# Vchitect/Latte

Hardware: AMD Instinct MI355X
Metric: denoising steps/sec (higher is better)
Workload: dtype f16; 1 GPU; Latte-XL/2 FaceForensics (uncond) 16x256x256 -> latents 16x4x32x32, DDIM on the '250' respacing, random-init weights; per_gpu_batch=8, global_batch=8, parallelism=dp1 (independent samples)

## Files before the change

### latte_amd/csrc/common.h

```cpp
#pragma once
#include <hip/hip_runtime.h>
#include <stdint.h>
#include <atomic>
#include <string>
#include <vector>

#include "../../include/latte_amd.h"

struct latte_schedule {
  int num_timesteps = 0;
  std::vector<int64_t> timestep_map;
  std::vector<double> betas, alphas_cumprod, alphas_cumprod_prev, alphas_cumprod_next, sqrt_recip_alphas_cumprod,
      sqrt_recipm1_alphas_cumprod, posterior_variance, posterior_log_variance_clipped, posterior_mean_coef1,
      posterior_mean_coef2, log_betas, sqrt_alphas_cumprod, sqrt_one_minus_alphas_cumprod;
  int mean_type = 0;
  int var_type = 0;
  mutable float* dev_tables = nullptr;
  mutable int dev_tables_device = -1;
};
enum DevTable : int { DT_SQRT_AC = 0, DT_SQRT_1MAC, DT_COEF1, DT_COEF2, DT_POST_LOGVAR, DT_LOG_BETAS, DT_SQRT_RECIP, DT_SQRT_RECIPM1,
                      DT_FIXED_LOGVAR, LATTE_NUM_DEV_TABLES };

extern "C" int schedule_device_tables(const latte_schedule_t* s, const float** out, hipStream_t st);

// ... 56 lines not shown
  int gate_stride;
  int rows_per_sample;
  int stagger;
  int group_m;
  int rmw_mode;
  int tag;
  int k_chunk;
  long split_stride;
  const uint8_t* A8;
  const uint8_t* W8;
  const uint8_t* A4;
  const uint8_t* W4;
  const uint8_t* A4s;
  const uint8_t* W4s;
  half_t* aux;
};
constexpr int LO8_A_SHIFT = 12, LO8_W_SHIFT = 6;
inline int lo4_pitch(int K) { return (K + 255) / 256 * 128; }
bool gemm_lo8_ok(int M, int N, int K);
bool gemm_lo4_ok(int M, int N, int K);
int launch_gemm(const GemmArgs& a, int epi, int dtype, int variant, hipStream_t st);
int launch_gemm_pw(const GemmArgs& a, int epi, int dtype, int roll, hipStream_t st);
int gemm_tile_m(int variant);
int gemm_tile_n(int variant);
int gemm_auto_variant(int M, int N, int epi);
int gemm_resolve_variant(int M, int N, int K, int epi);
bool gemm_small_tile_ok(int M, int N, int K);

struct AttnArgs {
  const half_t* qkv;
  half_t* out;
  int num_seq;
// ... 45 lines not shown
                       float* out, int BF, int C, int H, int p, int D, hipStream_t st);
int launch_final_layer(const float* x, const float* shift, const float* scale, int mod_stride,
                       const float* Wt , const float* bias, float* out, int M, int D,
                       int rows_per_sample, int T, int p, int Cout, int H, hipStream_t st);
int launch_cond_rows(const float* temb, const float* ytab, const int64_t* y, float* out, int n_steps, int bu, int D,
                     hipStream_t st);
int launch_text_proj(const float* text, const float* W, const float* bias, float* out, int B, int N, int K, hipStream_t st);
int launch_iota(int64_t* p, int n, hipStream_t st);
int launch_gated_split_reduce(float* x, const float* ws, int splits, size_t stride, const float* bias, const float* gate,
                              int gate_stride, int rows_per_sample, int M, int N, hipStream_t st);
int launch_silu_rows(const float* in, float* out, size_t n, hipStream_t st);
int launch_adaln_single(const float* tables , const float* head_table , const float* t6 ,
                        const float* temb , float* mod, int B, int nblk, int D, hipStream_t st);
int launch_permute_cf(const float* in, float* out, int B, int C, int F, int hw, int to_bfc, hipStream_t st);
int launch_fill_f32(float* p, float v, size_t n, hipStream_t st);
enum DebugChoice { DBG_ATTN_VARIANT = 0, DBG_XATTN_FLASH, DBG_TN_KERNEL, DBG_TN_WN, DBG_ATTN_BWD_TILES, DBG_CONV_KERNEL, DBG_VAE_SPLIT, DBG_NUM_CHOICES };
int debug_choice(DebugChoice c);
int set_debug_choice(const char* name, int value);

int launch_scale_f32(float* p, float s, size_t n, hipStream_t st);
int launch_scale_f32_dev(float* p, const float* s_dev, int inverse, size_t n, hipStream_t st);
int launch_t2v_guided_ddim(float* x, const float* model_out, int b, int C, int Cout, int F, int hw, float scale, float c1, float c2,
                           float c3, float c4, hipStream_t st);
struct T2VLinearStep {
  float scale, m_x, m_eps, c_x, c0, c1, c2, c3, c_noise, in_scale_next;
  int push;
};
int launch_t2v_guided_linear_step(float* x, float* x_in, const float* model_out, const float* h1, const float* h2, const float* h3,
                                  const float* noise, float* hw, int b, int C, int Cout, int F, int HW, const T2VLinearStep& s,
                                  hipStream_t st);
int launch_linear_step(float* x, float* x_in, const float* model_out, const float* h1, const float* h2, const float* h3,
// ... 159 lines not shown
```

### latte_amd/csrc/debug.hip

```cpp
#include "../../include/latte_amd_debug.h"
#include "common.h"

namespace {
typedef __attribute__((ext_vector_type(4))) __bf16 bf16x4;
__global__ void tr16_probe_kernel(uint16_t* out) {
  __shared__ __attribute__((aligned(16))) uint16_t lds[512];
  for (int i = threadIdx.x; i < 512; i += 64) lds[i] = (uint16_t)i;
  __syncthreads();
  const int lane = threadIdx.x;
  auto p = (__attribute__((address_space(3))) bf16x4*)((__attribute__((address_space(3))) char*)lds + 8 * lane);
  bf16x4 v = __builtin_amdgcn_ds_read_tr16_b64_v4bf16(p);
  typedef __attribute__((ext_vector_type(4))) unsigned short u16x4;
  u16x4 u = __builtin_bit_cast(u16x4, v);
  for (int j = 0; j < 4; ++j) out[lane * 4 + j] = u[j];
}

typedef __attribute__((address_space(3))) void lds_void_t;
__global__ void __launch_bounds__(512) dma_probe_kernel(const char* src, long long* out, int mode, int reps) {
  extern __shared__ __attribute__((aligned(16))) char smem[];
  const int lane = threadIdx.x & 63, wave = __builtin_amdgcn_readfirstlane(threadIdx.x >> 6);
  const __amdgpu_buffer_rsrc_t rs = __builtin_amdgcn_make_buffer_rsrc((void*)src, 0, 1u << 30, 0x00020000);
  char* my = smem + wave * 16384;
  const unsigned base = ((blockIdx.x & 63) * 8 + wave) * 16384u;
  long long t_issue = 0, t_all = 0;
// ... 96 lines not shown
extern "C" {

int latte_debug_dma_probe(const void* src_1gib_window, long long* out, int mode, int waves, int reps, void* stream) {
  if (waves < 1 || waves > 8) return fail(LATTE_ERR_INVALID, "dma_probe: waves must be 1..8");
  return launch_lds<dma_probe_kernel>(dim3(256), dim3(64 * waves), 8 * 16384, (hipStream_t)stream, (const char*)src_1gib_window, out, mode,
                                      reps);
}

int latte_debug_gemm(const void* A, const void* W, const float* bias, void* out, const float* gate, int M, int N, int K,
                     int gate_stride, int rows_per_sample, int epi, int dtype, int variant, void* stream) {
  GemmArgs g{};
  g.A = (const half_t*)A; g.W = (const half_t*)W; g.bias = bias; g.out = out; g.gate = gate;
  g.M = M; g.N = N; g.K = K; g.gate_stride = gate_stride; g.rows_per_sample = rows_per_sample;
  if (epi == EPI_BIAS_RES_H16) g.res = (const half_t*)gate;
  if (variant >= 1000) { g.tag = variant / 1000; variant %= 1000; }
  return launch_gemm(g, epi, dtype, variant, (hipStream_t)stream);
}

int latte_debug_gemm_gelu(const void* A, const void* W, const float* bias, void* out, void* aux, int M, int N, int K, int epi, int dtype,
                          void* stream) {
  if (epi != EPI_BIAS_GELU_DUAL_H16 && epi != EPI_DGELU_H16) return fail(LATTE_ERR_INVALID, "gemm_gelu: epi 13 (dual GELU) or 14 (dGELU)");
  GemmArgs g{};
  g.A = (const half_t*)A; g.W = (const half_t*)W; g.bias = bias; g.out = out; g.aux = (half_t*)aux;
  g.M = M; g.N = N; g.K = K; g.rows_per_sample = M;
  return launch_gemm_pw(g, epi, dtype, 1, (hipStream_t)stream);
}

int latte_debug_gemm_lo8(const void* A, const void* W, const void* A8, const void* W8, const float* bias, void* out, const float* gate,
                         int M, int N, int K, int gate_stride, int rows_per_sample, int epi, int dtype, void* stream) {
  if (!A8 || !W8) return fail(LATTE_ERR_INVALID, "gemm_lo8: null fp8 operand");
  GemmArgs g{};
  g.A = (const half_t*)A; g.W = (const half_t*)W; g.bias = bias; g.out = out; g.gate = gate;
  g.M = M; g.N = N; g.K = K; g.gate_stride = gate_stride; g.rows_per_sample = rows_per_sample;
  g.A8 = (const uint8_t*)A8; g.W8 = (const uint8_t*)W8;
  return launch_gemm(g, epi, dtype, 0, (hipStream_t)stream);
}

int latte_debug_gemm_lo4(const void* A, const void* W, const void* A4, const void* A4s, const void* W4, const void* W4s, const float* bias,
                         void* out, const float* gate, int M, int N, int K, int gate_stride, int rows_per_sample, int epi, int dtype,
                         void* stream) {
  if (!A4 || !A4s || !W4 || !W4s) return fail(LATTE_ERR_INVALID, "gemm_lo4: null fp4 operand");
  GemmArgs g{};
  g.A = (const half_t*)A; g.W = (const half_t*)W; g.bias = bias; g.out = out; g.gate = gate;
  g.M = M; g.N = N; g.K = K; g.gate_stride = gate_stride; g.rows_per_sample = rows_per_sample;
  g.A4 = (const uint8_t*)A4; g.A4s = (const uint8_t*)A4s; g.W4 = (const uint8_t*)W4; g.W4s = (const uint8_t*)W4s;
  return launch_gemm(g, epi, dtype, 0, (hipStream_t)stream);
}

int latte_debug_pack_w4(const void* w, void* out4, void* out_scale, int N, int K, int dtype, void* stream) {
  return launch_pack_w4((const half_t*)w, (unsigned char*)out4, (unsigned char*)out_scale, N, K, dtype, (hipStream_t)stream);
}

int latte_debug_ln_modulate_split4(const float* x, void* y, void* y4, void* y4s, const float* shift, const float* scale, int mod_stride, int M,
                                   int D, int rows_per_sample, int dtype, void* stream) {
  return launch_ln_modulate_split4(x, (half_t*)y, (unsigned char*)y4, (unsigned char*)y4s, shift, scale, mod_stride, M, D, rows_per_sample,
                                   dtype, (hipStream_t)stream);
}

int latte_debug_pack_w8(const void* w, void* out8, int64_t n, int dtype, void* stream) {
  return launch_pack_w8((const half_t*)w, (unsigned char*)out8, n, dtype, (hipStream_t)stream);
// ... 698 lines not shown
```

### latte_amd/csrc/engine.cpp

```cpp
#include <algorithm>
#include <cmath>
#include <cstdio>
#include <cstring>
#include <string>
#include <vector>

#include "event_profile.h"
#include "weight_store.h"

namespace latte {

static thread_local std::string g_last_error;
static std::atomic<int> g_debug_choice[DBG_NUM_CHOICES];
int debug_choice(DebugChoice c) { return g_debug_choice[c].load(std::memory_order_relaxed); }
int set_debug_choice(const char* name, int value) {
  static const char* const names[DBG_NUM_CHOICES] = {"attn_variant", "xattn_flash", "tn_kernel", "tn_wn", "attn_bwd_tiles", "conv_kernel", "vae_split"};
  static const int allowed[DBG_NUM_CHOICES][4] = {{1, 5, 12, 13}, {1, 0, 0, 0}, {4, 0, 0, 0}, {4, 0, 0, 0}, {1, 2, 0, 0}, {1, 2, 3, 4}, {0, 0, 0, 0}};
  for (int i = 0; i < DBG_NUM_CHOICES; ++i) {
    if (name && std::string(name) == names[i]) {
      bool ok = value == 0;
      for (int k = 0; k < 4; ++k) ok = ok || (allowed[i][k] != 0 && value == allowed[i][k]);
      ok = ok || (i == DBG_VAE_SPLIT && (value >> 24) == 1);
      if (!ok) return -1;
      g_debug_choice[i].store(value, std::memory_order_relaxed);
      return 0;
    }
  }
  return -1;
}
void set_error(const std::string& msg) { g_last_error = msg; }
int fail(int code, const std::string& msg) {
  g_last_error = msg;
// ... 12 lines not shown

}

using namespace latte;

struct latte_engine {
  latte_model_config_t cfg;
  int max_batch = 0;
  int D = 0, T = 0, F = 0, G = 0, Cin = 0, Cout = 0, H = 0, P = 0, KPE = 0, Hm = 0, hd = 0;
  int nmod = 0;
  int64_t rows_max = 0, rows_pad = 0;
  int gemm_variant = 0;
  int gemm_variant_of[4] = {0, 0, 0, 0};
  int fuse_qkv_attn = 3;
  int gated_split_k = 0;
  int guided_split = 20;
  int guided_split_active = 0;
  bool split_failed = false;
  bool split_w_ready = false;
  hipEvent_t load_event = nullptr;
  half_t* xn2 = nullptr;
  unsigned char* lo8 = nullptr;
  unsigned char *lo4 = nullptr, *lo4s = nullptr;
  float *split_ws = nullptr, *zero_bias = nullptr;
  std::vector<BlockW> blocks;
  float *ada_w = nullptr, *ada_b = nullptr, *pos = nullptr, *temp = nullptr, *pe_wt = nullptr, *pe_b = nullptr,
        *t0_w = nullptr, *t0_b = nullptr, *t2_w = nullptr, *t2_b = nullptr, *ytab = nullptr, *fin_wt = nullptr,
        *fin_b = nullptr;
  float *xres = nullptr, *mod = nullptr, *temb0 = nullptr, *cvec = nullptr, *model_out = nullptr, *noise_buf = nullptr;
  half_t *xn = nullptr, *qkv = nullptr, *hbuf = nullptr;
// ... 30 lines not shown
enum { C_QKV = 0, C_PROJ, C_FC1, C_FC2, C_ATTN_S, C_ATTN_T, C_LN, C_COND, C_PATCH, C_FINAL, C_QKVATTN_S, C_QKVATTN_T, C_NONE = -1 };

constexpr int64_t SPLIT_WS_FLOATS = 256ll * 256 * 192;
int gated_split_choice(const latte_engine* e, int M, int N, int K, int variant) {
  if (variant != 0 || e->gated_split_k == 1 || N % 192 || K % 64) return 1;
  if (e->gated_split_k == 0 && gemm_small_tile_ok(M, N, K)) return 1;
  const int tiles = ((M + 255) / 256) * (N / 192), nk = K / 64;
  if (e->gated_split_k >= 2) {
    const int s = e->gated_split_k;
    return (nk % s == 0 && (int64_t)s * M * N <= SPLIT_WS_FLOATS) ? s : 1;
  }
  for (int s = 4; s >= 2; --s)
    if (tiles * s <= 256 && nk % s == 0 && nk / s >= 32 && (int64_t)s * M * N <= SPLIT_WS_FLOATS) return s;
  return 1;
}
int gated_gemm(latte_engine* e, const GemmArgs& g, int dt, int variant, hipStream_t st) {
  if (g.A8) return launch_gemm(g, EPI_GATE_RES_F32, dt, 0, st);
  const int s = gated_split_choice(e, g.M, g.N, g.K, variant);
  if (s == 1) return launch_gemm(g, EPI_GATE_RES_F32, dt, variant, st);
  GemmArgs p = g;
  p.bias = e->zero_bias;
  p.gate = nullptr;
  p.out = e->split_ws;
  p.k_chunk = g.K / s;
  p.split_stride = (long)g.M * g.N;
  if (int rc = launch_gemm(p, EPI_BIAS_F32, dt, 5, st)) return rc;
  return launch_gated_split_reduce((float*)g.out, e->split_ws, s, (size_t)g.M * g.N, g.bias, g.gate, g.gate_stride,
                                   g.rows_per_sample, g.M, g.N, st);
}

// ... 88 lines not shown
  if ((gsplit & 16) && !gemm_lo4_ok(M, e->Hm, D)) gsplit = (gsplit & ~16) | 8;
  if (gsplit & 16) gsplit &= ~10;
  if (gsplit & 4) gsplit &= ~1;
  if (gsplit & 8) gsplit &= ~2;
  if ((gsplit & 4) && !gemm_lo8_ok(M, D, D)) gsplit = (gsplit & ~4) | 1;
  if ((gsplit & 8) && !gemm_lo8_ok(M, e->Hm, D)) gsplit = (gsplit & ~8) | 2;
  if ((gsplit & 3) && (uint64_t)e->rows_pad * 2 * D * 2 >= (1ull << 32)) gsplit &= ~3;
  if (gsplit) gsplit = ensure_split_weights(e, gsplit, st);
  int gactive = gsplit & 26;

  for (int i = 0; i < c.depth; ++i) {
    const bool spatial = (i % 2) == 0;
    const BlockW& w = e->blocks[i];
    const float* mb = modp + (size_t)i * 6 * D;
    bool split_proj = false;
    const float* te = (i == 1) ? e->temp : nullptr;
    if ((rc = launch_ln_modulate(e->xres, e->xres, e->xn, mb, mb + D, mstride, M, D, rps, te, T, F, dt, st))) return rc;
    tm.mark(C_LN);
    GemmArgs g{};
    g.M = M; g.rows_per_sample = rps; g.gate_stride = mstride;
    const half_t* attn_out = e->xn;
    if (((e->fuse_qkv_attn >> (spatial ? 0 : 1)) & 1) && qkv_attention_fusable(D, c.num_heads, e->hd, F, T, spatial ? 0 : 1, M)) {
      QkvAttnArgs qa{};
      qa.xn = e->xn; qa.w = w.qkv_w; qa.bias = w.qkv_b; qa.out = e->qkv; qa.B = B; qa.F = F; qa.T = T; qa.D = D;
      qa.heads = c.num_heads; qa.hd = e->hd; qa.mode = spatial ? 0 : 1; qa.scale = 1.0f / std::sqrt((float)e->hd);
      qa.flags = ((e->fuse_qkv_attn >> 2) & 7) ^ 7;
      split_proj = gsplit & 5;
      qa.out_split = (gsplit & 4) ? 2 : (gsplit & 1);
      qa.out8 = e->lo8;
      gactive |= gsplit & 5;
      if ((rc = launch_qkv_attention(qa, dt, st))) return rc;
      tm.mark(spatial ? C_QKVATTN_S : C_QKVATTN_T);
      attn_out = e->qkv;
    } else {
      g.A = e->xn; g.W = w.qkv_w; g.bias = w.qkv_b; g.out = e->qkv; g.N = 3 * D; g.K = D;
// ... 20 lines not shown
    tm.mark(C_PROJ);
    const int split_fc1 = (gsplit & 16) ? 3 : (gsplit & 8) ? 2 : (gsplit & 2) ? 1 : 0;
    if (split_fc1 == 3) rc = launch_ln_modulate_split4(e->xres, e->xn, e->lo4, e->lo4s, mb + 3 * D, mb + 4 * D, mstride, M, D, rps, dt, st);
    else rc = launch_ln_modulate(e->xres, e->xres, split_fc1 == 1 ? e->xn2 : e->xn, mb + 3 * D, mb + 4 * D, mstride, M, D, rps, nullptr, T, F, dt, st,
                                 split_fc1, e->lo8);
    if (rc) return rc;
    tm.mark(C_LN);
    g.A = e->xn; g.W = w.fc1_w; g.bias = w.fc1_b; g.out = e->hbuf; g.gate = nullptr; g.N = e->Hm; g.K = D;
    if (split_fc1 == 1) { g.A = e->xn2; g.W = w.fc1_w2; g.K = 2 * D; }
    if (split_fc1 == 2) { g.A8 = e->lo8; g.W8 = w.fc1_w8; }
    if (split_fc1 == 3) { g.A4 = e->lo4; g.A4s = e->lo4s; g.W4 = w.fc1_w4; g.W4s = w.fc1_w4s; }
    if ((rc = launch_gemm(g, EPI_BIAS_GELU_H16, dt, e->gemm_variant_of[2] ? e->gemm_variant_of[2] : e->gemm_variant, st))) return rc;
    g.A8 = nullptr; g.W8 = nullptr; g.A4 = nullptr; g.A4s = nullptr; g.W4 = nullptr; g.W4s = nullptr;
    tm.mark(C_FC1);
    g.A = e->hbuf; g.W = w.fc2_w; g.bias = w.fc2_b; g.out = e->xres; g.gate = mb + 5 * D; g.N = D; g.K = e->Hm; g.tag = 1;

    if ((rc = gated_gemm(e, g, dt, e->gemm_variant_of[3] ? e->gemm_variant_of[3] : e->gemm_variant, st))) return rc;
    tm.mark(C_FC2);
  }
  const float* fm = modp + (size_t)c.depth * 6 * D;
  if ((rc = launch_final_layer(e->xres, fm, fm + D, mstride, e->fin_wt, e->fin_b, out, M, D, rps, T, c.patch_size,
                               e->Cout, e->H, st))) return rc;
  tm.mark(C_FINAL);
  if (cfg_dup) e->guided_split_active = gactive;
  return LATTE_OK;
}

int grow(latte_engine* e, float** p, int64_t* cap, int64_t need) {
  if (*cap >= need) return LATTE_OK;
  if (*p) {
    e->arena.release(*p);
    *p = nullptr;
// ... 260 lines not shown
    return LATTE_OK;
  }
  for (int gi = 0; gi < 4; ++gi) {
    static const char* names[4] = {"gemm_variant_qkv", "gemm_variant_proj", "gemm_variant_fc1", "gemm_variant_fc2"};
    if (k == names[gi]) {
      if (value < 0 || (value > 13 && value != 18 && value != 19)) return fail(LATTE_ERR_INVALID, "gemm_variant_*: must be 0..13, 18 or 19");
      e->gemm_variant_of[gi] = (int)value;
      return LATTE_OK;
    }
  }
  if (k == "gated_split_k") {
    if (value < 0 || value > 4) return fail(LATTE_ERR_INVALID, "gated_split_k: 0 (rule), 1 (off) or 2..4 splits");
    e->gated_split_k = (int)value;
    return LATTE_OK;
  }
  if (k == "fuse_qkv_attn") {
    if (value < 0 || value > 31)
      return fail(LATTE_ERR_INVALID, "fuse_qkv_attn: bit 0 = spatial blocks, bit 1 = temporal blocks, bits 2-4 = schedule features off (0..31)");
    e->fuse_qkv_attn = (int)value;
    return LATTE_OK;
  }
  if (k == "guided_split") {
    if (value < 0 || value > 31)
      return fail(LATTE_ERR_INVALID, "guided_split: bit 0 / 1 = attention output / fc1 operand as f16 split pairs, bit 2 / 3 = the same with an fp8 remainder, bit 4 = fc1's operand with an fp4 remainder, in guided calls (0..31)");
    e->guided_split = (int)value;
    return LATTE_OK;
  }
  if (k == "seed") {
    e->seed = (uint64_t)value;
    e->rng_offset = 0;
// ... 4 lines not shown
    e->train_timesteps = (int)value;
    return LATTE_OK;
  }
  return fail(LATTE_ERR_INVALID, "set_option: unknown option '" + k + "'");
}

int latte_engine_get_option(const latte_engine_t* e, const char* name, int64_t* value) {
  if (!e || !name || !value) return fail(LATTE_ERR_INVALID, "get_option: null argument");
  const std::string k = name;
  if (k == "gemm_variant") *value = e->gemm_variant;
  else if (k == "gemm_variant_qkv") *value = e->gemm_variant_of[0];
  else if (k == "gemm_variant_proj") *value = e->gemm_variant_of[1];
  else if (k == "gemm_variant_fc1") *value = e->gemm_variant_of[2];
  else if (k == "gemm_variant_fc2") *value = e->gemm_variant_of[3];
  else if (k == "gated_split_k") *value = e->gated_split_k;
  else if (k == "fuse_qkv_attn") *value = e->fuse_qkv_attn;
  else if (k == "guided_split") *value = e->guided_split;
  else if (k == "guided_split_active") *value = e->guided_split_active;
  else if (k == "guided_split_failed") *value = e->split_failed ? 1 : 0;
  else if (k == "seed") *value = (int64_t)e->seed;
  else if (k == "train_timesteps") *value = e->train_timesteps;
  else return fail(LATTE_ERR_INVALID, "get_option: unknown option '" + k + "'");
  return LATTE_OK;
}

int latte_engine_load_tensor(latte_engine_t* e, const char* key, const float* data, int64_t numel, int on_device,
                             void* stream) {
  if (!e || !key || !data) return fail(LATTE_ERR_INVALID, "load_tensor: null argument");
  hipStream_t st = (hipStream_t)stream;
  WeightSlot* slot = nullptr;
// ... 544 lines not shown
```

### latte_amd/csrc/gemm.hip

```cpp
#include <type_traits>

#include "common.h"
#include "mfma_util.h"

namespace latte {
namespace {

template <int EPI, int DT>
__device__ __forceinline__ void epilogue_store(const GemmArgs& g, const f32x4& a, int m, int n, const float* gate_row) {
  const float4 b4 = *(const float4*)(g.bias + n);
  float v0 = a[0] + b4.x, v1 = a[1] + b4.y, v2 = a[2] + b4.z, v3 = a[3] + b4.w;
  const size_t o = (size_t)m * g.N + n;
  if constexpr (EPI == EPI_BIAS_RES_H16) {
    const u32x2 r2 = *(const u32x2*)(g.res + o);
    if constexpr (DT == LATTE_DTYPE_BF16) {
      v0 += __builtin_bit_cast(float, r2[0] << 16); v1 += __builtin_bit_cast(float, r2[0] & 0xffff0000u);
      v2 += __builtin_bit_cast(float, r2[1] << 16); v3 += __builtin_bit_cast(float, r2[1] & 0xffff0000u);
    } else {
      const unsigned int lo = r2[0], hi = r2[1];
      v0 += (float)__builtin_bit_cast(_Float16, (unsigned short)(lo & 0xffffu));
      v1 += (float)__builtin_bit_cast(_Float16, (unsigned short)(lo >> 16));
      v2 += (float)__builtin_bit_cast(_Float16, (unsigned short)(hi & 0xffffu));
      v3 += (float)__builtin_bit_cast(_Float16, (unsigned short)(hi >> 16));
    }
// ... 791 lines not shown
  return variant;
}

int launch_gemm(const GemmArgs& a_in, int epi, int dtype, int variant, hipStream_t st) {
  GemmArgs a = a_in;
  if (a.group_m == 0 && epi == EPI_GATE_RES_F32) a.group_m = 4;
  if (a.A4) {
    if (!gemm_lo4_ok(a.M, a.N, a.K)) return fail(LATTE_ERR_INVALID, "gemm: the fp4 correction pass needs N % 192 == 0, K % 64 == 0, K >= 128");
    return launch_gemm_pw(a, epi, dtype, 1, st);
  }
  if (a.A8) {
    if (!gemm_lo8_ok(a.M, a.N, a.K)) return fail(LATTE_ERR_INVALID, "gemm: the fp8 correction pass needs N % 192 == 0 and K % 128 == 0");
    return launch_gemm_pw(a, epi, dtype, 1, st);
  }
  if (variant == 0) variant = gemm_resolve_variant(a.M, a.N, a.K, epi);
  if (variant == 10 || variant == 11) return launch_gemm_pw(a, epi, dtype, variant == 11, st);
  const int bn = gemm_tile_n(variant);
  const int nq = variant >= 7 && variant <= 9 ? bn / 4 : bn;
  if (a.K % 64 != 0 || a.N % nq != 0 || a.M <= 0)
    return fail(LATTE_ERR_INVALID, "gemm: shape not tileable (need K % 64 == 0, N % tileN == 0)");
  if (dtype == LATTE_DTYPE_BF16) return launch_dt<LATTE_DTYPE_BF16>(a, epi, variant, st);
  if (dtype == LATTE_DTYPE_F16) return launch_dt<LATTE_DTYPE_F16>(a, epi, variant, st);
  return fail(LATTE_ERR_INVALID, "gemm: unknown dtype");
}

}
```

### latte_amd/csrc/gemm_pw.hip

```cpp
#include <type_traits>

#include "common.h"
#include "mfma_util.h"

namespace latte {
namespace {

template <int DT>
__device__ __forceinline__ void mfma16_ip(f32x4& c, const u32x4& a, const u32x4& b) {
  if constexpr (DT == LATTE_DTYPE_BF16)
    asm volatile("v_mfma_f32_16x16x32_bf16 %0, %1, %2, %0" : "+v"(c) : "v"(a), "v"(b));
  else
    asm volatile("v_mfma_f32_16x16x32_f16 %0, %1, %2, %0" : "+v"(c) : "v"(a), "v"(b));
}

template <int DT>
__device__ __forceinline__ void mfma16_first(f32x4& c, const u32x4& a, const u32x4& b) {
  if constexpr (DT == LATTE_DTYPE_BF16)
    asm volatile("v_mfma_f32_16x16x32_bf16 %0, %1, %2, 0" : "=v"(c) : "v"(a), "v"(b));
  else
    asm volatile("v_mfma_f32_16x16x32_f16 %0, %1, %2, 0" : "=v"(c) : "v"(a), "v"(b));
}

typedef __attribute__((ext_vector_type(8))) unsigned int u32x8;
__device__ __forceinline__ u32x8 cat8(const u32x4& lo, const u32x4& hi) { return __builtin_shufflevector(lo, hi, 0, 1, 2, 3, 4, 5, 6, 7); }
__device__ __forceinline__ void mfma8_ip(f32x4& c, const u32x8& a, const u32x8& b, unsigned sa, unsigned sb) {
  asm volatile("v_mfma_scale_f32_16x16x128_f8f6f4 %0, %1, %2, %0, %3, %4 op_sel_hi:[0,0,0]" : "+v"(c) : "v"(a), "v"(b), "v"(sa), "v"(sb));
}

template <int N> __device__ __forceinline__ void wait_vm() { asm volatile("s_waitcnt vmcnt(%0)" ::"n"(N) : "memory"); }

template <int EPI, int DT, int TAG>
__global__ void __launch_bounds__(768) gemm_pw_kernel(GemmArgs g) {
  constexpr int BM = 256, BN = 192, FN = 3, WTN = 48;
  constexpr int A_BYTES = BM * 128, B_BYTES = BN * 128;
  constexpr int NA = 3;
  constexpr int B_BASE = NA * A_BYTES;
  constexpr int AH_INSTR = 4, BG_INSTR = 6;
  constexpr int GROUP_M = 8;

  extern __shared__ __attribute__((aligned(16))) char smem[];
  const int lane = threadIdx.x & 63;
// ... 203 lines not shown
        for (int j = 0; j < FN; ++j) acc[i][j] = mfma16<DT>(bf[1][j], af[i], acc[i][j]);
      }
      __builtin_amdgcn_s_setprio(0);
      if (grp == 1 && last) epilogue(tm, tn);
      __builtin_amdgcn_s_barrier();
      if (grp == 0 && last) epilogue(tm, tn);
    }
    pos += per;
    if (pos >= cnt) break;
    decode(chunk0 + pos, tm, tn);
  }
  if (grp == 0) __builtin_amdgcn_s_barrier();
}


template <int EPI, int DT, int TAG, int LO = 0>
__global__ void __launch_bounds__(768) gemm_pwr_kernel(GemmArgs g) {
  constexpr int BM = 256, BN = 192, FN = 3, WTN = 48;
  constexpr int A_BYTES = BM * 128, B_BYTES = BN * 128;
  constexpr int NA = 3;
  constexpr int B_BASE = NA * A_BYTES;
  constexpr int AH_INSTR = 4, BG_INSTR = 6;
  constexpr int GROUP_M = 8;
  constexpr int PATCH_BYTES = 16 * 112;

  extern __shared__ __attribute__((aligned(16))) char smem[];
  const int lane = threadIdx.x & 63;
  const int wave = __builtin_amdgcn_readfirstlane(threadIdx.x >> 6);
  const int K = g.K;
  const unsigned row_bytes = (unsigned)K * 2u;

// ... 170 lines not shown
          }
        }
        if constexpr (EPI == EPI_BIAS_GELU_DUAL_H16) {
#pragma unroll
          for (int j = 0; j < FN; ++j) *(u32x2*)(patch + fr * 112 + j * 32 + gq * 8) = side[j];
          const u32x4 w0 = *(const u32x4*)(patch + r0 * 112 + p0 * 16);
          if (m0_ < g.M) *(u32x4*)(g.aux + (size_t)m0_ * g.N + ncol0 + p0 * 8) = w0;
          if (le < 32) {
            const u32x4 w1 = *(const u32x4*)(patch + r1 * 112 + p1 * 16);
            if (m1_ < g.M) *(u32x4*)(g.aux + (size_t)m1_ * g.N + ncol0 + p1 * 8) = w1;
          }
        }
      }
      return;
    }
    if constexpr (EPI == EPI_GATE_RES_F32) {
      if ((g.rows_per_sample % BM) == 0) {
        float* const outp = (float*)g.out;
        const float* gr = g.gate + (size_t)((tm_ * BM) / g.rows_per_sample) * g.gate_stride + ncol;
        float4 b4[FN], g1[FN];
#pragma unroll
        for (int j = 0; j < FN; ++j) {
          b4[j] = *(const float4*)(g.bias + ncol + j * 16);
          g1[j] = *(const float4*)(gr + j * 16);
        }
        constexpr int NF = 8 * FN, AHEAD = 2;
        auto frag_ptr = [&](int f) -> float* {
          const int mc = min(mbase + (f / FN) * 16, g.M - 1);
          return outp + (size_t)mc * g.N + ncol + (f % FN) * 16;
        };
        float4 qa[AHEAD];
#pragma unroll
        for (int a = 0; a < AHEAD; ++a) qa[a] = *(const float4*)frag_ptr(a);
#pragma unroll
        for (int f = 0; f < NF; ++f) {
          float4 rr = qa[f % AHEAD];
          if (f + AHEAD < NF) qa[f % AHEAD] = *(const float4*)frag_ptr(f + AHEAD);
          asm volatile("" ::: "memory");
          const int i = f / FN, j = f % FN;
          rr.x += g1[j].x * (acc[i][j][0] + b4[j].x);
          rr.y += g1[j].y * (acc[i][j][1] + b4[j].y);
          rr.z += g1[j].z * (acc[i][j][2] + b4[j].z);
          rr.w += g1[j].w * (acc[i][j][3] + b4[j].w);
          if (mbase + i * 16 < g.M) *(float4*)(outp + (size_t)(mbase + i * 16) * g.N + ncol + j * 16) = rr;
          acc[i][j] = (f32x4){0.f, 0.f, 0.f, 0.f};
        }
        return;
      }
    }
#pragma unroll
    for (int i = 0; i < 8; ++i) {
      const int m = mbase + i * 16;
      if (m < g.M) {
#pragma unroll
        for (int j = 0; j < FN; ++j) {
          const int n = ncol + j * 16;
          const float4 b4 = *(const float4*)(g.bias + n);
          float v0 = acc[i][j][0] + b4.x, v1 = acc[i][j][1] + b4.y, v2 = acc[i][j][2] + b4.z, v3 = acc[i][j][3] + b4.w;
          const size_t o = (size_t)m * g.N + n;
          if constexpr (EPI == EPI_GATE_RES_F32) {
            const float4 g4 = *(const float4*)(g.gate + (size_t)(m / g.rows_per_sample) * g.gate_stride + n);
            float4* dst = (float4*)((float*)g.out + o);
            float4 rr = *dst;
            rr.x += g4.x * v0; rr.y += g4.y * v1; rr.z += g4.z * v2; rr.w += g4.w * v3;
            *dst = rr;
          } else if constexpr (EPI == EPI_BIAS_F32) {
            *(float4*)((float*)g.out + o) = make_float4(v0, v1, v2, v3);
          } else {
            if constexpr (EPI == EPI_BIAS_GELU_H16) {
              auto gelu = [](float x) {
                const float p = __builtin_fmaf(x * x, -0.10294324f, -2.3022082f);
                return x * __builtin_amdgcn_rcpf(1.0f + __builtin_amdgcn_exp2f(p * x));
              };
              v0 = gelu(v0); v1 = gelu(v1); v2 = gelu(v2); v3 = gelu(v3);
            }
            const u32x2 p = {pack2<DT>(v0, v1), pack2<DT>(v2, v3)};
            *(u32x2*)((half_t*)g.out + o) = p;
          }
        }
// ... 236 lines not shown
        lo_tile(sA8, nullptr, nullptr, std::false_type{});
        ++it;
      }
      asm volatile("s_nop 15\n\ts_nop 15" ::: "memory");
      epilogue(tm, tn);
    }
    pos += per;
    if (pos >= cnt) break;
    decode(chunk0 + pos, tm, tn);
    fill(smem + ia * A_BYTES, smem + (it & 1) * B_BYTES);
  }
}



template <int EPI, int DT, int TAG>
int launch_pw_roll(const GemmArgs& a, int roll, dim3 grid, dim3 block, int lds, hipStream_t st) {
  if (roll) return launch_lds<gemm_pwr_kernel<EPI, DT, TAG>>(grid, block, lds, st, a);
  return launch_lds<gemm_pw_kernel<EPI, DT, TAG>>(grid, block, lds, st, a);
}

template <int DT>
int launch_pw_dt(const GemmArgs& a, int epi, int roll, hipStream_t st) {
  constexpr int LDS = 3 * 256 * 128 + 2 * 192 * 128 + 8 * 16 * 112;
  const int tiles = ((a.M + 255) / 256) * (a.N / 192);
  const int nblk = tiles >= 256 ? 256 : (tiles + 7) / 8 * 8;
  dim3 grid(nblk), block(768);
  if (a.A4) {
    if (!roll || !a.W4 || !a.A4s || !a.W4s || !(epi == EPI_GATE_RES_F32 || epi == EPI_BIAS_GELU_H16) || DT != LATTE_DTYPE_F16)
      return fail(LATTE_ERR_INVALID, "gemm: the fp4 correction pass needs the rolling kernel, f16 operands, both code images with their row scales, and the gated / GELU epilogue");
    if constexpr (DT == LATTE_DTYPE_F16) {
      const bool half_tail = (a.K & 255) != 0 && (a.K & 255) <= 128;
      if (epi == EPI_GATE_RES_F32)
        return half_tail ? launch_lds<gemm_pwr_kernel<EPI_GATE_RES_F32, DT, 0, 3>>(grid, block, LDS, st, a)
                         : launch_lds<gemm_pwr_kernel<EPI_GATE_RES_F32, DT, 0, 2>>(grid, block, LDS, st, a);
      return half_tail ? launch_lds<gemm_pwr_kernel<EPI_BIAS_GELU_H16, DT, 0, 3>>(grid, block, LDS, st, a)
                       : launch_lds<gemm_pwr_kernel<EPI_BIAS_GELU_H16, DT, 0, 2>>(grid, block, LDS, st, a);
    }
    return LATTE_OK;
  }
  if (a.A8) {
    if (!roll || !a.W8 || a.K % 128 != 0 || !(epi == EPI_GATE_RES_F32 || epi == EPI_BIAS_GELU_H16) || DT != LATTE_DTYPE_F16)
      return fail(LATTE_ERR_INVALID, "gemm (correction pass): rolling kernel, f16 operands, K % 128 == 0, gated-residual or GELU epilogue only");
    if constexpr (DT == LATTE_DTYPE_F16) {
      if (epi == EPI_GATE_RES_F32) return launch_lds<gemm_pwr_kernel<EPI_GATE_RES_F32, DT, 0, 1>>(grid, block, LDS, st, a);
      return launch_lds<gemm_pwr_kernel<EPI_BIAS_GELU_H16, DT, 0, 1>>(grid, block, LDS, st, a);
    }
    return LATTE_OK;
  }
  switch (epi) {
    case EPI_GATE_RES_F32:
      if (a.tag == 1) return launch_pw_roll<EPI_GATE_RES_F32, DT, 1>(a, roll, grid, block, LDS, st);
      return launch_pw_roll<EPI_GATE_RES_F32, DT, 0>(a, roll, grid, block, LDS, st);
    case EPI_BIAS_F32: return launch_pw_roll<EPI_BIAS_F32, DT, 0>(a, roll, grid, block, LDS, st);
    case EPI_BIAS_H16: return launch_pw_roll<EPI_BIAS_H16, DT, 0>(a, roll, grid, block, LDS, st);
    case EPI_BIAS_GELU_H16: return launch_pw_roll<EPI_BIAS_GELU_H16, DT, 0>(a, roll, grid, block, LDS, st);
    case EPI_BIAS_GELU_DUAL_H16:
    case EPI_DGELU_H16:
      if (!roll || !a.aux) return fail(LATTE_ERR_INVALID, "gemm (producer-wave kernel): the GELU training epilogues need the rolling kernel and GemmArgs::aux");
      if (epi == EPI_BIAS_GELU_DUAL_H16) return launch_lds<gemm_pwr_kernel<EPI_BIAS_GELU_DUAL_H16, DT, 0>>(grid, block, LDS, st, a);
      return launch_lds<gemm_pwr_kernel<EPI_DGELU_H16, DT, 0>>(grid, block, LDS, st, a);
    default: return fail(LATTE_ERR_INVALID, "gemm (producer-wave kernel): unknown epilogue");
  }
}

}
// ... 22 lines not shown
```

Measured before the change: 259.9 sample-steps/s.

## Add line-wise gated residual RMW epilogue and fuse temp_embed into first fc2

Adds a new gated-residual epilogue variant (RS=1) for the rolling 12-wave GEMM. It uses DPP row rotations to regroup accumulator fragments, so residual reads and writes cover contiguous lines instead of scattered fragments. This mode is the new default. It also moves the temporal-embedding addition from the second block's LayerNorm pass into block 0's fc2 epilogue (TAG=2) when that GEMM uses variant 11 without split-K, which avoids an extra read of the embedding in the LN kernel. Both paths add more template instantiations and new cross-lane shuffle logic that could raise register pressure.

```diff
diff --git a/latte_amd/csrc/common.h b/latte_amd/csrc/common.h
--- a/latte_amd/csrc/common.h
+++ b/latte_amd/csrc/common.h
@@ -94,8 +94,11 @@
   const uint8_t* A4s;
   const uint8_t* W4s;
   half_t* aux;
+  const float* te;
+  int te_T, te_F;
 };
 constexpr int LO8_A_SHIFT = 12, LO8_W_SHIFT = 6;
+constexpr int GATED_RMW_SHAPE_DEFAULT = 1;
 inline int lo4_pitch(int K) { return (K + 255) / 256 * 128; }
 bool gemm_lo8_ok(int M, int N, int K);
 bool gemm_lo4_ok(int M, int N, int K);
@@ -171,7 +174,7 @@
                         const float* temb , float* mod, int B, int nblk, int D, hipStream_t st);
 int launch_permute_cf(const float* in, float* out, int B, int C, int F, int hw, int to_bfc, hipStream_t st);
 int launch_fill_f32(float* p, float v, size_t n, hipStream_t st);
-enum DebugChoice { DBG_ATTN_VARIANT = 0, DBG_XATTN_FLASH, DBG_TN_KERNEL, DBG_TN_WN, DBG_ATTN_BWD_TILES, DBG_CONV_KERNEL, DBG_VAE_SPLIT, DBG_NUM_CHOICES };
+enum DebugChoice { DBG_ATTN_VARIANT = 0, DBG_XATTN_FLASH, DBG_TN_KERNEL, DBG_TN_WN, DBG_ATTN_BWD_TILES, DBG_CONV_KERNEL, DBG_VAE_SPLIT, DBG_GATED_RMW_SHAPE, DBG_NUM_CHOICES };
 int debug_choice(DebugChoice c);
 int set_debug_choice(const char* name, int value);
 
diff --git a/latte_amd/csrc/debug.hip b/latte_amd/csrc/debug.hip
--- a/latte_amd/csrc/debug.hip
+++ b/latte_amd/csrc/debug.hip
@@ -134,6 +134,8 @@
   g.M = M; g.N = N; g.K = K; g.gate_stride = gate_stride; g.rows_per_sample = rows_per_sample;
   if (epi == EPI_BIAS_RES_H16) g.res = (const half_t*)gate;
   if (variant >= 1000) { g.tag = variant / 1000; variant %= 1000; }
+  const int shape = debug_choice(DBG_GATED_RMW_SHAPE);
+  g.rmw_mode = shape ? shape - 1 : GATED_RMW_SHAPE_DEFAULT;
   return launch_gemm(g, epi, dtype, variant, (hipStream_t)stream);
 }
 
@@ -153,6 +155,8 @@
   g.A = (const half_t*)A; g.W = (const half_t*)W; g.bias = bias; g.out = out; g.gate = gate;
   g.M = M; g.N = N; g.K = K; g.gate_stride = gate_stride; g.rows_per_sample = rows_per_sample;
   g.A8 = (const uint8_t*)A8; g.W8 = (const uint8_t*)W8;
+  const int shape = debug_choice(DBG_GATED_RMW_SHAPE);
+  g.rmw_mode = shape ? shape - 1 : GATED_RMW_SHAPE_DEFAULT;
   return launch_gemm(g, epi, dtype, 0, (hipStream_t)stream);
 }
 
@@ -164,6 +168,8 @@
   g.A = (const half_t*)A; g.W = (const half_t*)W; g.bias = bias; g.out = out; g.gate = gate;
   g.M = M; g.N = N; g.K = K; g.gate_stride = gate_stride; g.rows_per_sample = rows_per_sample;
   g.A4 = (const uint8_t*)A4; g.A4s = (const uint8_t*)A4s; g.W4 = (const uint8_t*)W4; g.W4s = (const uint8_t*)W4s;
+  const int shape = debug_choice(DBG_GATED_RMW_SHAPE);
+  g.rmw_mode = shape ? shape - 1 : GATED_RMW_SHAPE_DEFAULT;
   return launch_gemm(g, epi, dtype, 0, (hipStream_t)stream);
 }
 
diff --git a/latte_amd/csrc/engine.cpp b/latte_amd/csrc/engine.cpp
--- a/latte_amd/csrc/engine.cpp
+++ b/latte_amd/csrc/engine.cpp
@@ -14,8 +14,8 @@
 static std::atomic<int> g_debug_choice[DBG_NUM_CHOICES];
 int debug_choice(DebugChoice c) { return g_debug_choice[c].load(std::memory_order_relaxed); }
 int set_debug_choice(const char* name, int value) {
-  static const char* const names[DBG_NUM_CHOICES] = {"attn_variant", "xattn_flash", "tn_kernel", "tn_wn", "attn_bwd_tiles", "conv_kernel", "vae_split"};
-  static const int allowed[DBG_NUM_CHOICES][4] = {{1, 5, 12, 13}, {1, 0, 0, 0}, {4, 0, 0, 0}, {4, 0, 0, 0}, {1, 2, 0, 0}, {1, 2, 3, 4}, {0, 0, 0, 0}};
+  static const char* const names[DBG_NUM_CHOICES] = {"attn_variant", "xattn_flash", "tn_kernel", "tn_wn", "attn_bwd_tiles", "conv_kernel", "vae_split", "gated_rmw_shape"};
+  static const int allowed[DBG_NUM_CHOICES][4] = {{1, 5, 12, 13}, {1, 0, 0, 0}, {4, 0, 0, 0}, {4, 0, 0, 0}, {1, 2, 0, 0}, {1, 2, 3, 4}, {0, 0, 0, 0}, {1, 2, 0, 0}};
   for (int i = 0; i < DBG_NUM_CHOICES; ++i) {
     if (name && std::string(name) == names[i]) {
       bool ok = value == 0;
@@ -58,6 +58,8 @@
   int gemm_variant_of[4] = {0, 0, 0, 0};
   int fuse_qkv_attn = 3;
   int gated_split_k = 0;
+  int gated_rmw_shape = GATED_RMW_SHAPE_DEFAULT;
+  int fc2_temp_embed = 1;
   int guided_split = 20;
   int guided_split_active = 0;
   bool split_failed = false;
@@ -118,6 +120,10 @@
     if (tiles * s <= 256 && nk % s == 0 && nk / s >= 32 && (int64_t)s * M * N <= SPLIT_WS_FLOATS) return s;
   return 1;
 }
+bool gated_gemm_takes_te(const latte_engine* e, int M, int N, int K, int variant) {
+  if (gated_split_choice(e, M, N, K, variant) != 1) return false;
+  return (variant ? variant : gemm_resolve_variant(M, N, K, EPI_GATE_RES_F32)) == 11;
+}
 int gated_gemm(latte_engine* e, const GemmArgs& g, int dt, int variant, hipStream_t st) {
   if (g.A8) return launch_gemm(g, EPI_GATE_RES_F32, dt, 0, st);
   const int s = gated_split_choice(e, g.M, g.N, g.K, variant);
@@ -236,11 +242,13 @@
     const BlockW& w = e->blocks[i];
     const float* mb = modp + (size_t)i * 6 * D;
     bool split_proj = false;
-    const float* te = (i == 1) ? e->temp : nullptr;
+    const int fc2_variant = e->gemm_variant_of[3] ? e->gemm_variant_of[3] : e->gemm_variant;
+    const bool te_in_fc2 = e->fc2_temp_embed && c.depth > 1 && gated_gemm_takes_te(e, M, D, e->Hm, fc2_variant);
+    const float* te = (i == 1 && !te_in_fc2) ? e->temp : nullptr;
     if ((rc = launch_ln_modulate(e->xres, e->xres, e->xn, mb, mb + D, mstride, M, D, rps, te, T, F, dt, st))) return rc;
     tm.mark(C_LN);
     GemmArgs g{};
-    g.M = M; g.rows_per_sample = rps; g.gate_stride = mstride;
+    g.M = M; g.rows_per_sample = rps; g.gate_stride = mstride; g.rmw_mode = e->gated_rmw_shape;
     const half_t* attn_out = e->xn;
     if (((e->fuse_qkv_attn >> (spatial ? 0 : 1)) & 1) && qkv_attention_fusable(D, c.num_heads, e->hd, F, T, spatial ? 0 : 1, M)) {
       QkvAttnArgs qa{};
@@ -291,8 +299,8 @@
     g.A8 = nullptr; g.W8 = nullptr; g.A4 = nullptr; g.A4s = nullptr; g.W4 = nullptr; g.W4s = nullptr;
     tm.mark(C_FC1);
     g.A = e->hbuf; g.W = w.fc2_w; g.bias = w.fc2_b; g.out = e->xres; g.gate = mb + 5 * D; g.N = D; g.K = e->Hm; g.tag = 1;
-
-    if ((rc = gated_gemm(e, g, dt, e->gemm_variant_of[3] ? e->gemm_variant_of[3] : e->gemm_variant, st))) return rc;
+    if (i == 0 && te_in_fc2) { g.te = e->temp; g.te_T = T; g.te_F = F; }
+    if ((rc = gated_gemm(e, g, dt, fc2_variant, st))) return rc;
     tm.mark(C_FC2);
   }
   const float* fm = modp + (size_t)c.depth * 6 * D;
@@ -583,6 +591,16 @@
     e->gated_split_k = (int)value;
     return LATTE_OK;
   }
+  if (k == "gated_rmw_shape") {
+    if (value < 0 || value > 1) return fail(LATTE_ERR_INVALID, "gated_rmw_shape: 0 (fragment-wise) or 1 (line-wise residual accesses of the gated GEMMs)");
+    e->gated_rmw_shape = (int)value;
+    return LATTE_OK;
+  }
+  if (k == "fc2_temp_embed") {
+    if (value < 0 || value > 1) return fail(LATTE_ERR_INVALID, "fc2_temp_embed: 0 (LayerNorm pass adds temp_embed) or 1 (the first block's fc2 epilogue does)");
+    e->fc2_temp_embed = (int)value;
+    return LATTE_OK;
+  }
   if (k == "fuse_qkv_attn") {
     if (value < 0 || value > 31)
       return fail(LATTE_ERR_INVALID, "fuse_qkv_attn: bit 0 = spatial blocks, bit 1 = temporal blocks, bits 2-4 = schedule features off (0..31)");
@@ -617,6 +635,8 @@
   else if (k == "gemm_variant_fc1") *value = e->gemm_variant_of[2];
   else if (k == "gemm_variant_fc2") *value = e->gemm_variant_of[3];
   else if (k == "gated_split_k") *value = e->gated_split_k;
+  else if (k == "gated_rmw_shape") *value = e->gated_rmw_shape;
+  else if (k == "fc2_temp_embed") *value = e->fc2_temp_embed;
   else if (k == "fuse_qkv_attn") *value = e->fuse_qkv_attn;
   else if (k == "guided_split") *value = e->guided_split;
   else if (k == "guided_split_active") *value = e->guided_split_active;
diff --git a/latte_amd/csrc/gemm.hip b/latte_amd/csrc/gemm.hip
--- a/latte_amd/csrc/gemm.hip
+++ b/latte_amd/csrc/gemm.hip
@@ -829,6 +829,8 @@
     return launch_gemm_pw(a, epi, dtype, 1, st);
   }
   if (variant == 0) variant = gemm_resolve_variant(a.M, a.N, a.K, epi);
+  if (a.te && !(variant == 11 && epi == EPI_GATE_RES_F32))
+    return fail(LATTE_ERR_INVALID, "gemm: GemmArgs::te exists in the rolling 12-wave kernel's gated epilogue only (variant 11)");
   if (variant == 10 || variant == 11) return launch_gemm_pw(a, epi, dtype, variant == 11, st);
   const int bn = gemm_tile_n(variant);
   const int nq = variant >= 7 && variant <= 9 ? bn / 4 : bn;
diff --git a/latte_amd/csrc/gemm_pw.hip b/latte_amd/csrc/gemm_pw.hip
--- a/latte_amd/csrc/gemm_pw.hip
+++ b/latte_amd/csrc/gemm_pw.hip
@@ -26,6 +26,11 @@
 __device__ __forceinline__ u32x8 cat8(const u32x4& lo, const u32x4& hi) { return __builtin_shufflevector(lo, hi, 0, 1, 2, 3, 4, 5, 6, 7); }
 __device__ __forceinline__ void mfma8_ip(f32x4& c, const u32x8& a, const u32x8& b, unsigned sa, unsigned sb) {
   asm volatile("v_mfma_scale_f32_16x16x128_f8f6f4 %0, %1, %2, %0, %3, %4 op_sel_hi:[0,0,0]" : "+v"(c) : "v"(a), "v"(b), "v"(sa), "v"(sb));
+}
+
+template <int BANKS>
+__device__ __forceinline__ float ror8(float old, float src) {
+  return __int_as_float(__builtin_amdgcn_update_dpp(__float_as_int(old), __float_as_int(src), 0x128, 0xf, BANKS, false));
 }
 
 template <int N> __device__ __forceinline__ void wait_vm() { asm volatile("s_waitcnt vmcnt(%0)" ::"n"(N) : "memory"); }
@@ -259,7 +264,7 @@
 }
 
 
-template <int EPI, int DT, int TAG, int LO = 0>
+template <int EPI, int DT, int TAG, int LO = 0, int RS = 0>
 __global__ void __launch_bounds__(768) gemm_pwr_kernel(GemmArgs g) {
   constexpr int BM = 256, BN = 192, FN = 3, WTN = 48;
   constexpr int A_BYTES = BM * 128, B_BYTES = BN * 128;
@@ -460,7 +465,64 @@
       }
       return;
     }
-    if constexpr (EPI == EPI_GATE_RES_F32) {
+    auto te_ptr = [&](int m_clamped, int n) -> const float* {
+      return g.te + (size_t)((m_clamped / g.te_T) % g.te_F) * g.N + n;
+    };
+    static_assert(!(TAG == 2 && RS == 1), "the temporal-embedding epilogue has the fragment-wise form only");
+    if constexpr (EPI == EPI_GATE_RES_F32 && RS == 1) {
+      if ((g.rows_per_sample % BM) == 0) {
+        float* const outp = (float*)g.out;
+        const bool odd = wn & 1;
+        const int gq = le >> 4;
+        const int n0 = tn_ * BN + wn * WTN;
+        const int nline = n0 + (odd ? 16 : 0) + ((fr >> 3) * 4 + gq) * 4;
+        const int nhalf = n0 + (odd ? 0 : 32) + gq * 4;
+        const int mline = tm_ * BM + grp * 128 + (fr & 7);
+        const float* gs = g.gate + (size_t)((tm_ * BM) / g.rows_per_sample) * g.gate_stride;
+        const float4 gl = *(const float4*)(gs + nline), gh = *(const float4*)(gs + nhalf);
+        float4 b4[FN];
+#pragma unroll
+        for (int j = 0; j < FN; ++j) b4[j] = *(const float4*)(g.bias + ncol + j * 16);
+        constexpr int NQ = 8 * 3, AHEAD = 2;
+        auto row_of = [&](int q) -> int { return (q % 3 == 2 ? mbase : mline + (q % 3) * 8) + (q / 3) * 16; };
+        auto col_of = [&](int q) -> int { return q % 3 == 2 ? nhalf : nline; };
+        float4 qa[AHEAD];
+        auto load = [&](int q) {
+          const int mc = min(row_of(q), g.M - 1);
+          qa[q % AHEAD] = *(const float4*)(outp + (size_t)mc * g.N + col_of(q));
+        };
+#pragma unroll
+        for (int a = 0; a < AHEAD; ++a) load(a);
+        f32x4 t[3];
+#pragma unroll
+        for (int q = 0; q < NQ; ++q) {
+          float4 rr = qa[q % AHEAD];
+          if (q + AHEAD < NQ) load(q + AHEAD);
+          asm volatile("" ::: "memory");
+          const int i = q / 3, k = q % 3;
+          if (k == 0) {
+            f32x4 s[FN];
+#pragma unroll
+            for (int j = 0; j < FN; ++j) {
+              s[j] = (f32x4){acc[i][j][0] + b4[j].x, acc[i][j][1] + b4[j].y, acc[i][j][2] + b4[j].z, acc[i][j][3] + b4[j].w};
+              acc[i][j] = (f32x4){0.f, 0.f, 0.f, 0.f};
+            }
+            const f32x4 l0 = odd ? s[1] : s[0], l1 = odd ? s[2] : s[1];
+            t[2] = odd ? s[0] : s[2];
+            t[0] = (f32x4){ror8<0xC>(l0[0], l1[0]), ror8<0xC>(l0[1], l1[1]), ror8<0xC>(l0[2], l1[2]), ror8<0xC>(l0[3], l1[3])};
+            t[1] = (f32x4){ror8<0x3>(l1[0], l0[0]), ror8<0x3>(l1[1], l0[1]), ror8<0x3>(l1[2], l0[2]), ror8<0x3>(l1[3], l0[3])};
+          }
+          const float4 gg = k == 2 ? gh : gl;
+          rr.x = __builtin_fmaf(gg.x, t[k][0], rr.x);
+          rr.y = __builtin_fmaf(gg.y, t[k][1], rr.y);
+          rr.z = __builtin_fmaf(gg.z, t[k][2], rr.z);
+          rr.w = __builtin_fmaf(gg.w, t[k][3], rr.w);
+          if (row_of(q) < g.M) *(float4*)(outp + (size_t)row_of(q) * g.N + col_of(q)) = rr;
+        }
+        return;
+      }
+    }
+    if constexpr (EPI == EPI_GATE_RES_F32 && RS == 0) {
       if ((g.rows_per_sample % BM) == 0) {
         float* const outp = (float*)g.out;
         const float* gr = g.gate + (size_t)((tm_ * BM) / g.rows_per_sample) * g.gate_stride + ncol;
@@ -475,19 +537,25 @@
           const int mc = min(mbase + (f / FN) * 16, g.M - 1);
           return outp + (size_t)mc * g.N + ncol + (f % FN) * 16;
         };
-        float4 qa[AHEAD];
-#pragma unroll
-        for (int a = 0; a < AHEAD; ++a) qa[a] = *(const float4*)frag_ptr(a);
+        float4 qa[AHEAD], qe[AHEAD];
+        auto load_te = [&](int f) {
+          if constexpr (TAG == 2) qe[f % AHEAD] = *(const float4*)te_ptr(min(mbase + (f / FN) * 16, g.M - 1), ncol + (f % FN) * 16);
+        };
+#pragma unroll
+        for (int a = 0; a < AHEAD; ++a) { qa[a] = *(const float4*)frag_ptr(a); load_te(a); }
 #pragma unroll
         for (int f = 0; f < NF; ++f) {
           float4 rr = qa[f % AHEAD];
-          if (f + AHEAD < NF) qa[f % AHEAD] = *(const float4*)frag_ptr(f + AHEAD);
+          float4 e4 = make_float4(0.f, 0.f, 0.f, 0.f);
+          if constexpr (TAG == 2) e4 = qe[f % AHEAD];
+          if (f + AHEAD < NF) { qa[f % AHEAD] = *(const float4*)frag_ptr(f + AHEAD); load_te(f + AHEAD); }
           asm volatile("" ::: "memory");
           const int i = f / FN, j = f % FN;
           rr.x += g1[j].x * (acc[i][j][0] + b4[j].x);
           rr.y += g1[j].y * (acc[i][j][1] + b4[j].y);
           rr.z += g1[j].z * (acc[i][j][2] + b4[j].z);
           rr.w += g1[j].w * (acc[i][j][3] + b4[j].w);
+          if constexpr (TAG == 2) { rr.x += e4.x; rr.y += e4.y; rr.z += e4.z; rr.w += e4.w; }
           if (mbase + i * 16 < g.M) *(float4*)(outp + (size_t)(mbase + i * 16) * g.N + ncol + j * 16) = rr;
           acc[i][j] = (f32x4){0.f, 0.f, 0.f, 0.f};
         }
@@ -509,6 +577,10 @@
             float4* dst = (float4*)((float*)g.out + o);
             float4 rr = *dst;
             rr.x += g4.x * v0; rr.y += g4.y * v1; rr.z += g4.z * v2; rr.w += g4.w * v3;
+            if constexpr (TAG == 2) {
+              const float4 e4 = *(const float4*)te_ptr(m, n);
+              rr.x += e4.x; rr.y += e4.y; rr.z += e4.z; rr.w += e4.w;
+            }
             *dst = rr;
           } else if constexpr (EPI == EPI_BIAS_F32) {
             *(float4*)((float*)g.out + o) = make_float4(v0, v1, v2, v3);
@@ -775,9 +847,19 @@
 
 
 
+template <int DT, int TAG, int LO>
+int launch_pwr_gated(const GemmArgs& a, dim3 grid, dim3 block, int lds, hipStream_t st) {
+  if (a.rmw_mode) return launch_lds<gemm_pwr_kernel<EPI_GATE_RES_F32, DT, TAG, LO, 1>>(grid, block, lds, st, a);
+  return launch_lds<gemm_pwr_kernel<EPI_GATE_RES_F32, DT, TAG, LO, 0>>(grid, block, lds, st, a);
+}
+
 template <int EPI, int DT, int TAG>
 int launch_pw_roll(const GemmArgs& a, int roll, dim3 grid, dim3 block, int lds, hipStream_t st) {
-  if (roll) return launch_lds<gemm_pwr_kernel<EPI, DT, TAG>>(grid, block, lds, st, a);
+  if constexpr (EPI == EPI_GATE_RES_F32) {
+    if (roll) return launch_pwr_gated<DT, TAG, 0>(a, grid, block, lds, st);
+  } else {
+    if (roll) return launch_lds<gemm_pwr_kernel<EPI, DT, TAG>>(grid, block, lds, st, a);
+  }
   return launch_lds<gemm_pw_kernel<EPI, DT, TAG>>(grid, block, lds, st, a);
 }
 
@@ -787,14 +869,14 @@
   const int tiles = ((a.M + 255) / 256) * (a.N / 192);
   const int nblk = tiles >= 256 ? 256 : (tiles + 7) / 8 * 8;
   dim3 grid(nblk), block(768);
+  if ((a.A4 || a.A8) && a.te) return fail(LATTE_ERR_INVALID, "gemm: GemmArgs::te has no correction-pass form");
   if (a.A4) {
     if (!roll || !a.W4 || !a.A4s || !a.W4s || !(epi == EPI_GATE_RES_F32 || epi == EPI_BIAS_GELU_H16) || DT != LATTE_DTYPE_F16)
       return fail(LATTE_ERR_INVALID, "gemm: the fp4 correction pass needs the rolling kernel, f16 operands, both code images with their row scales, and the gated / GELU epilogue");
     if constexpr (DT == LATTE_DTYPE_F16) {
       const bool half_tail = (a.K & 255) != 0 && (a.K & 255) <= 128;
       if (epi == EPI_GATE_RES_F32)
-        return half_tail ? launch_lds<gemm_pwr_kernel<EPI_GATE_RES_F32, DT, 0, 3>>(grid, block, LDS, st, a)
-                         : launch_lds<gemm_pwr_kernel<EPI_GATE_RES_F32, DT, 0, 2>>(grid, block, LDS, st, a);
+        return half_tail ? launch_pwr_gated<DT, 0, 3>(a, grid, block, LDS, st) : launch_pwr_gated<DT, 0, 2>(a, grid, block, LDS, st);
       return half_tail ? launch_lds<gemm_pwr_kernel<EPI_BIAS_GELU_H16, DT, 0, 3>>(grid, block, LDS, st, a)
                        : launch_lds<gemm_pwr_kernel<EPI_BIAS_GELU_H16, DT, 0, 2>>(grid, block, LDS, st, a);
     }
@@ -804,13 +886,17 @@
     if (!roll || !a.W8 || a.K % 128 != 0 || !(epi == EPI_GATE_RES_F32 || epi == EPI_BIAS_GELU_H16) || DT != LATTE_DTYPE_F16)
       return fail(LATTE_ERR_INVALID, "gemm (correction pass): rolling kernel, f16 operands, K % 128 == 0, gated-residual or GELU epilogue only");
     if constexpr (DT == LATTE_DTYPE_F16) {
-      if (epi == EPI_GATE_RES_F32) return launch_lds<gemm_pwr_kernel<EPI_GATE_RES_F32, DT, 0, 1>>(grid, block, LDS, st, a);
+      if (epi == EPI_GATE_RES_F32) return launch_pwr_gated<DT, 0, 1>(a, grid, block, LDS, st);
       return launch_lds<gemm_pwr_kernel<EPI_BIAS_GELU_H16, DT, 0, 1>>(grid, block, LDS, st, a);
     }
     return LATTE_OK;
   }
   switch (epi) {
     case EPI_GATE_RES_F32:
+      if (a.te) {
+        if (!roll || a.te_T <= 0 || a.te_F <= 0) return fail(LATTE_ERR_INVALID, "gemm (producer-wave kernel): GemmArgs::te needs the rolling kernel and te_T, te_F > 0");
+        return launch_lds<gemm_pwr_kernel<EPI_GATE_RES_F32, DT, 2, 0, 0>>(grid, block, LDS, st, a);
+      }
       if (a.tag == 1) return launch_pw_roll<EPI_GATE_RES_F32, DT, 1>(a, roll, grid, block, LDS, st);
       return launch_pw_roll<EPI_GATE_RES_F32, DT, 0>(a, roll, grid, block, LDS, st);
     case EPI_BIAS_F32: return launch_pw_roll<EPI_BIAS_F32, DT, 0>(a, roll, grid, block, LDS, st);
```

New measurement: 262.5 sample-steps/s (median of 6 runs). 1.01x the previous value.
